# labgem/pangenomeNEM

Hardware: AMD Instinct MI355X
Metric: em_family_x_organism_cells_per_sec (higher is better)
Workload: dtype f32 chains with f64 intermediates (reference arithmetic); int32 popcounts in the M-step; 1 GPU; BASELINE configs[1]: 20000 families x 500 organisms, K=3, beta=0.5, contiguity graph (path + 5% chords, weights 1..8), ncem/sk_/pk; U-shaped family-frequency spectrum (Beta(0.3, 0.3) per family), default .m init; families_total=20000, families_per_gpu=20000, organisms=500, K=3, parallelism=1 GPU

## Files before the change

pangenomenem_amd/csrc/nem_engine.hip:

```cpp
#include <hip/hip_runtime.h>
#include <dlfcn.h>
#include <pthread.h>
#include <unistd.h>

#include <algorithm>
#include <climits>
#include <atomic>
#include <cfloat>
#include <chrono>
#include <cmath>
#include <cstdio>
#include <cstdlib>
#include <cstring>
#include <condition_variable>
#include <deque>
#include <functional>
#include <map>
#include <string>
#include <mutex>
#include <thread>
#include <vector>

#include "nem_internal.hpp"
#include "nem_ff.hpp"
// ... 142 lines not shown
    int* stats_last = nullptr;
    float* par_copy[3] = {}; double* pkfki_copy[3] = {}; float* logpkfki_copy[3] = {};
    int round_batch = 3;
    int rounds_iter = 2;
    int deep_iters = 2;
    uint8_t fz_need[kFzPositions] = {}; uint8_t fz_init_need = 0;
    int run_deep_used = 0; bool run_tracked = false;
    bool capture_first = false;
    int n_plain = 0, n_captured = 0, n_replayed = 0, n_host_rounds = 0;
    int ff_mode = -1;
    bool fused_update() const
    {
        return d <= kFusedMaxD && (cfg.disper == NEMGPU_DISP_KD || cfg.disper == NEMGPU_DISP_K_);
    }
    bool use_ff() const { return ff_mode < 0 ? d >= 256 : ff_mode != 0; }
    bool fault_seen = false; int fault_inject = 0;

    hipEvent_t ev0 = nullptr, ev1 = nullptr;
    hipEvent_t ev_flags = nullptr;
    bool defer_layout = false, layout_pending = false;
    hipEvent_t ready_ev = nullptr;
    bool ready_pending = false;

    struct Chunk { char* base; size_t size, used; bool owned = true; };
    std::vector<Chunk> chunks;
    int shared_chunk = -1;
    uint8_t* best_lab = nullptr; float* best_c = nullptr;
    uint32_t* xf_stage = nullptr;
    bool ctrl_pending = false; CtrlArgs ctrl_deferred{};
    nemgpu_engine* parent = nullptr;
// ... 386 lines not shown
FinishArgs finish_args(nemgpu_engine* e, int mode, const int* stats)
{
    FinishArgs t;
    t.mode = mode;
    t.K = e->k; t.D = e->d; t.dpad = e->dpad; t.n_total = e->n_true; t.disper = e->cfg.disper; t.propor = e->cfg.propor;
    t.stats = stats; t.stats_ranks = 1; t.stats_rank_stride = 0;
    t.prop = e->prop; t.center = e->center; t.disp = e->disp; t.nbobs_k = e->nbobs_k; t.iner = e->iner;
    t.tabT = e->tabT; t.tabL0 = e->tabL0; t.nz0 = e->nz0; t.nz1 = e->nz1;
    t.am0 = e->am0; t.am1 = e->am1; t.uni = e->uni; t.nonuni = e->nonuni;
    t.pk = e->pk; t.logpk = e->logpk; t.flags = e->iter_flags();
    t.stop = e->stop_ptr;
    t.reset_prop = nullptr; t.reset_center = nullptr; t.reset_disp = nullptr;
    t.reset_ctrl = nullptr; t.reset_ctrl_words = 0; t.reset_sweep_next = nullptr;
    t.prev_center = nullptr; t.prev_disp = nullptr;
    t.zero_stats = nullptr; t.n_zero_stats = 0;
    t.use_ff = e->use_ff() ? 1 : 0;
    t.perm = e->perm;
    t.ffq = e->ffq;
    return t;
}

int do_tables(nemgpu_engine* e)
{
    if (e->tables_fresh) return NEMGPU_OK;
    launch_finish(finish_args(e, 0, nullptr), e->stream);
    HIPCHK(hipGetLastError());
    e->tables_fresh = true;
    e->density_fresh = false;
    return NEMGPU_OK;
}

// ... 1626 lines not shown
    e->wf = (d + 31) / 32;
    e->nw64 = (e->n + 63) / 64;
    e->cfg.algo = NEMGPU_ALGO_NCEM; e->cfg.beta = 0.5f; e->cfg.disper = NEMGPU_DISP_K_; e->cfg.propor = NEMGPU_PROP_K;
    e->cfg.cvtest = NEMGPU_CV_CLAS; e->cfg.cvthres = 1e-8f; e->cfg.it_max = 100; e->cfg.param_fix = 0;
    e->cfg.tie_rule = NEMGPU_TIE_HASH; e->cfg.tie_seed = 0;
    if (const char* g = getenv("NEM_MI355X_GRAPHS")) e->use_graphs = (g[0] != '0');
    if (const char* g = getenv("NEM_MI355X_SHADOW_VERIFY")) e->shadow_verify = (g[0] != '0');
    e->flag_sets = e->shadow_verify ? 3 : 1;
    if (const char* g = getenv("NEM_MI355X_ROUND_COUNTS")) e->round_counts = (g[0] != '0');
    if (const char* g = getenv("NEM_MI355X_START_FUSED")) e->start_fused = (g[0] != '0');
    if (const char* g = getenv("NEM_MI355X_ROUNDS")) e->round_batch = std::max(2, std::min(kRoundBatchMax, atoi(g)));
    if (const char* g = getenv("NEM_MI355X_ROUNDS_ITER")) e->rounds_iter = std::max(2, std::min(e->round_batch, atoi(g)));
    e->rounds_iter = std::min(e->rounds_iter, e->round_batch);
    if (const char* g = getenv("NEM_MI355X_FAULT_INJECT")) e->fault_inject = !strcmp(g, "fuzzy_pc") ? 1 : 0;
    if (const char* g = getenv("NEM_MI355X_FF")) e->ff_mode = (g[0] == '0') ? 0 : (g[0] == '1') ? 1 : -1;
    if (const char* g = getenv("NEM_MI355X_SORT")) e->use_sort = (g[0] != '0');
    if (hip_stream) { e->stream = (hipStream_t)hip_stream; e->own_stream = false; }
    else {
        if (pool_stream_get(device, &e->stream) != hipSuccess) { delete e; set_error("hipStreamCreate failed"); return NEMGPU_E_DEVICE; }
        e->own_stream = true;
    }
    int r = NEMGPU_OK;
    alloc_for(e);
    auto A = [&](int rr) { if (r == NEMGPU_OK) r = rr; };
    A(dev_alloc(&e->xw, (size_t)e->W * e->npad));
    A(dev_alloc(&e->xws, (size_t)((e->W + 3) / 4) * 4 * e->npad));
    A(dev_alloc(&e->perm, (size_t)e->npad));
    A(dev_alloc(&e->xt, (size_t)d * e->nw64));
    A(alloc_model_buffers(e));
    if (r == NEMGPU_OK && !e->flags_host &&
// ... 1612 lines not shown
    }
    if (best_start) *best_start = best;
    cleanup();
    return NEMGPU_OK;
}

static int make_clone(nemgpu_engine* p, nemgpu_engine** out, char* slab, size_t slab_bytes, int* flags_host, float* par0)
{
    nemgpu_engine* c = new nemgpu_engine();
    c->n_total = p->n_total; c->n_true = p->n_true; c->d = p->d; c->k = p->k; c->lo = p->lo; c->hi = p->hi; c->n = p->n;
    c->npad = p->npad; c->dpad = p->dpad; c->W = p->W; c->wf = p->wf; c->nw64 = p->nw64; c->device = p->device;
    c->stream = p->stream; c->own_stream = false;
    c->cfg = p->cfg; c->have_matrix = true; c->have_params = true; c->has_graph = p->has_graph;
    c->xw = p->xw; c->xws = p->xws; c->perm = p->perm; c->xt = p->xt; c->use_sort = p->use_sort;
    c->nei_ptr = p->nei_ptr; c->nei_idx = p->nei_idx; c->nei_w = p->nei_w; c->nnz = p->nnz;
    c->use_graphs = p->use_graphs; c->ff_mode = p->ff_mode; c->round_batch = p->round_batch; c->rounds_iter = p->rounds_iter;
    c->parent = p; c->carve_all = true;
    c->chunks.push_back({slab, slab_bytes, 0, false});
    c->shared_chunk = 0;
    c->flags_host = flags_host; c->flags_host_borrowed = true;
    const size_t kd = (size_t)p->k * p->d;
    c->prop0 = par0; c->center0 = par0 + p->k; c->disp0 = par0 + p->k + kd;
    alloc_for(c);
    int r = alloc_model_buffers(c);
    if (r == NEMGPU_OK) r = ensure_state_buffers(c);
    if (r == NEMGPU_OK) r = ensure_crit_buffers(c);
    alloc_for(p);
    if (r != NEMGPU_OK) { nemgpu_destroy(c); return r; }
    c->draw_ctl = c->sweep_next + 8;
    *out = c;
    return NEMGPU_OK;
// ... 63 lines not shown
        if (!e->libc()) { *out = rng.integer(mini, maxi); return NEMGPU_OK; }
        uint32_t v = 0;
        int rr = host_draw(e, &v);
        *out = (int)(v % (uint32_t)(maxi - mini + 1)) + mini;
        return rr;
    };
    auto bit = [&](int i, int j) { return (float)((e->host_bits[(size_t)i * wf + (j >> 5)] >> (j & 31)) & 1u); };
    alloc_for(e);
    if (e->ncem()) { if (!e->best_lab && (r = dev_alloc(&e->best_lab, (size_t)e->n_total))) return r; }
    else { if (!e->best_c && (r = dev_alloc(&e->best_c, (size_t)e->n_total * k))) return r; }
    const int group = std::min(n_starts, 64);
    const char* fa = getenv("NEM_MI355X_STARTS_FIRST_ALONE");
    int width = (e->libc() && !(fa && fa[0] == '0') && fn == nullptr) ? 1 : group;
    int voided_in_a_row = 0, clean_run = 0; bool alone_for_good = false;
    if ((r = ensure_clones(e, group))) return r;
    for (nemgpu_engine* c : e->clones) { c->cfg = e->cfg; c->stream = e->stream; c->round_batch = e->round_batch; c->ff_mode = e->ff_mode; }

    e->rs_rounds = e->rs_lockstep = e->rs_alone = e->rs_redone = e->rs_two_waits = 0;
    if (e->libc()) e->tie_heavy = true;
    int nbsucc = 0, best = -1, last_status = NEMGPU_OK;
    float best_crit[6] = {0, 0, 0, 0, 0, 0};
    nemgpu_result best_res{};
    std::vector<float> host_par;
    std::vector<int> start_pos;
    std::vector<GlibcRandom> rng_after;
    int next = 0;
    static const bool prof = getenv("NEM_MI355X_BATCH_PROF") != nullptr;
    while (next < n_starts) {
        const int M = std::min(width, n_starts - next);
        std::vector<nemgpu_engine*> E(e->clones.begin(), e->clones.begin() + M);
        host_par.assign((size_t)M * par, 0.0f);
// ... 1284 lines not shown
```

pangenomenem_amd/csrc/nem_kernels.hip:

```cpp
#include <hip/hip_runtime.h>
#include <cstdlib>
#include <algorithm>
#include <cfloat>
#include <cstdint>
#include <cstring>
#include <type_traits>

#include "nem_ff.hpp"
#include "nem_chain.hpp"
#include "nem_halfsum.hpp"
#include "nem_kernels.hpp"
#include "nem_sweep_dev.hpp"

namespace nemk {

#ifdef NEM_PHASE_PROF
__device__ unsigned long long g_phase[32];
#define NEM_PHASE(i) do { if (blockIdx.x == 0 && threadIdx.x == 0) g_phase[i] = wall_clock64(); } while (0)
#define NEM_PHASE_TAKE(t) const unsigned long long t = wall_clock64()
#define NEM_PHASE_PUT(i, t) do { if (blockIdx.x == 0 && threadIdx.x == 0) g_phase[i] = t; } while (0)
#else
#define NEM_PHASE(i) do { } while (0)
#define NEM_PHASE_TAKE(t) do { } while (0)
#define NEM_PHASE_PUT(i, t) do { } while (0)
#endif


__device__ __forceinline__ int stat_sum(const int* __restrict__ stats, int idx, int ranks, int stride)
{
    int s = stats[idx];
    for (int r = 1; r < ranks; r++) s += stats[idx + r * stride];
    return s;
}

__device__ inline int wave_reduce_add(int v)
{
// ... 234 lines not shown
    const uint32_t hi = ((mm >> j) & 1u) << 30;
    const double f = __hiloint2double((int)hi, 0);
    return __float_as_uint((float)(fma(f, l1h, (double)__uint_as_float(bits)) - l0));
}

__device__ __forceinline__ void ff_word(uint32_t& bits, uint32_t& q0, uint32_t& dq, uint32_t& end, uint32_t m, int nb,
                                        const uint32_t* sQ0, const uint32_t* sDQ, double l1h, double l0)
{
    const uint32_t cand = ff_cand(m, dq, (nb == 32) ? bits + (q0 << 5) : mad24((uint32_t)nb, q0, bits));
    const bool cross = cand >= end;
    bits = cross ? bits : cand;
    if (cross) {
        uint32_t mm = m;
        int rem = nb;
        for (;;) {
            uint32_t j = 0, at = bits;
#pragma unroll
            for (int sh = 4; sh >= 0; sh--) {
                const uint32_t t = j + (1u << sh);
                const uint32_t at_t = at + (q0 << sh);
                const bool fits = ff_probe(mm, t, dq, at_t) < end;
                j = fits ? t : j;
                at = fits ? at_t : at;
            }
            bits = ff_probe(mm, j, dq, at);
            bits = ff_exact_step(bits, mm, j, l1h, l0);
            ff_load(sQ0, sDQ, bits, q0, dq, end);
            rem -= (int)j + 1;
            if (rem <= 0) break;
            mm = mm >> (j + 1u);
// ... 52 lines not shown
    if (g < gfull) { ff_group(x0, g, am, bits, q0, q1, end, sQ0, sQ1, l1h, l0); xt = x1; g++; }
    if (g < gfull) { ff_group(x1, g, am, bits, q0, q1, end, sQ0, sQ1, l1h, l0); xt = x2; g++; }
    if (g < gfull) { ff_group(x2, g, am, bits, q0, q1, end, sQ0, sQ1, l1h, l0); xt = x3; g++; }
#pragma unroll
    for (int c = 0; c < 4; c++) {
        const int w = 4 * gfull + c;
        if (w > wlast) break;
        uint32_t m = mismatch_word(word_of(xt, c), am[w]);
        const int nb = (w < wlast) ? 32 : (D - (wlast << 5));
        if (nb < 32) m &= (1u << nb) - 1u;
        ff_word(bits, q0, q1, end, m, nb, sQ0, sQ1, l1h, l0);
    }
    return __uint_as_float(bits);
}

__device__ __forceinline__ void ff_build(uint32_t* sQ0, uint32_t* sDQ, double l1, double l0, int tid)
{
    uint32_t q0, q1;
    ff_entry(l1, -l0, tid, q0, q1);
    if (q0 == kFFInvalid) q1 = kFFInvalid;
    sQ0[tid] = q0; sDQ[tid] = q1 - q0;
}

__device__ __forceinline__ void density_store(const int* __restrict__ perm, int slot, int tile, int tid, int n, int npad, int k,
                                              float dk, uint32_t nul, double pk, float logpk,
                                              double* __restrict__ pkfki, float* __restrict__ logpkfki)
{
    __shared__ double sPk[256];
    __shared__ float sLp[256];
    float logfk; double fk;
// ... 99 lines not shown
    const float* center_in; const float* disp_in;
    int* iter_flags;
    double* pkfki; float* logpkfki;
    int* zero_flags; int n_zero_flags;
    int* zero_stats; int n_zero_stats;
    const int* stop;
    int use_ff;
    const int* perm;
};

struct StartArgs {
    const float* prop0; const float* center0; const float* disp0;
    int* ctrl; int ctrl_words; int* sweep_next;
};

template <bool START = false>
__device__ __forceinline__ int density_fused_body(const FusedDensityArgs& a, const StartArgs* st = nullptr)
{
    __shared__ __align__(16) float sVal[FD_MAXD];
    __shared__ double2 sT[FD_CH];
    __shared__ double sL[FD_CH];
    __shared__ uint2 sAm[FD_MAXD / 32];
    __shared__ uint32_t sNz0[FD_CH / 32], sNz1[FD_CH / 32];
    __shared__ uint32_t sQ0[256], sQ1[256];
    __shared__ unsigned long long sTot2w[4];
    __shared__ float sChain[2];
    __shared__ int sGenW[4];
    int k, tile;
    if (!density_tile(a.K, a.npad >> 8, tile, k)) return -1;
    const int tid = threadIdx.x, lane = tid & 63;
    const int i = tile * 256 + tid;
// ... 149 lines not shown
    uint32_t nul = 0;
    bool uniform = !eps_per_d && !any_general && ((double)eps_u > kEpsilonD);
    double l1 = 0.0, l0 = 0.0;
    if (uniform) {
        l1 = log((double)((1.0f - eps_u) / eps_u));
        l0 = log((double)(1.0f - eps_u));
        if (!isfinite(l1) || !isfinite(l0)) uniform = false;
    }
    if (uniform) {
        const double l1h = 0.5 * l1;
        if (a.use_ff && l1 >= 0.0 && l0 <= 0.0) {
            ff_build(sQ0, sQ1, l1, l0, tid);
            __syncthreads();
            NEM_PHASE(21);
            if constexpr (START) xh = xw_head(a.xw, npad, i, D);
            dk = chain_ff(xh, npad, D, sAm, sQ0, sQ1, l1h, l0);
        } else {
            if constexpr (START) xh = xw_head(a.xw, npad, i, D);
            dk = chain_plain(a.xw, xh, npad, i, D, sAm, l1h, l0);
        }
        NEM_PHASE(22);
    } else {
        const bool by_mask = nonempty && !any_general;
        const float* mu_in = START ? st->center0 : a.center_in;
        for (int d0 = 0; d0 < dpad; d0 += FD_CH) {
            const int dn = min(FD_CH, dpad - d0);
            __syncthreads();
            for (int t = tid; t < dn; t += 256) {
                const int d = d0 + t;
                double t0 = 0.0, t1 = 0.0, ll0 = 0.0;
                int n0 = 0, n1 = 0;
// ... 1168 lines not shown
bool launch_halfsum_debug(const float* x, int n, int waves, float* out, hipStream_t s, long long* stamps)
{
    if (n < 0 || n > kHalfsumDebugCap) return false;
    if (waves == 16) hipLaunchKernelGGL(k_halfsum_debug<16>, dim3(1), dim3(1024), 0, s, x, n, out, stamps);
    else if (waves == 1) hipLaunchKernelGGL(k_halfsum_debug<1>, dim3(1), dim3(64), 0, s, x, n, out, stamps);
    else return false;
    return true;
}


__global__ __launch_bounds__(1024) void k_finish(FinishArgs a) { finish_body(a, gridDim.x); }
__global__ __launch_bounds__(1024) void k_finish_b(const void* arr, int stride, const int* gx) { NEM_B_HEAD(FinishArgs) finish_body(a, nblk); }
__global__ __launch_bounds__(256) void k_density(DensityArgs a) { density_body(a); }
__global__ __launch_bounds__(256) void k_density_b(const void* arr, int stride, const int* gx) { NEM_B_HEAD(DensityArgs) density_body(a); }
__global__ __launch_bounds__(256) void k_density_fused(FusedDensityArgs a) { (void)density_fused_body(a); }
__global__ __launch_bounds__(256) void k_density_fused_b(const void* arr, int stride, const int* gx) { NEM_B_HEAD(FusedDensityArgs) (void)density_fused_body(a); }
__global__ __launch_bounds__(256) void k_density_start(FusedDensityArgs a, StartArgs st) { (void)density_fused_body<true>(a, &st); }
template <int KT, int R>
__global__ __launch_bounds__(256) void k_sweep_counts(SweepArgs s, CountsArgs c, int nsweep)
{
    if ((int)blockIdx.x < nsweep) { sweep_body<KT, true, 256, false>(s, blockIdx.x, nsweep); return; }
    mstep_counts_body<R>(c.K, c.D, c.nw64, c.xt, c.mask, c.stats, c.stop, CtrlArgs{}, (int)blockIdx.x - nsweep, (int)gridDim.x - nsweep);
}

template <int KT>
__global__ __launch_bounds__(256) void k_density_verify(FusedDensityArgs d, SweepArgs s, int nd)
{
    if ((int)blockIdx.x < nd) { (void)density_fused_body(d); return; }
    sweep_body<KT, true, 256, false>(s, (int)blockIdx.x - nd, (int)gridDim.x - nd);
}

__global__ void k_ctrl(CtrlArgs a) { ctrl_logic(a); }
// ... 133 lines not shown
    hipLaunchKernelGGL(k_finish, grid, dim3(1024), 0, s, a);
}

void launch_density(const FinishArgs& t, const uint32_t* xw, int n, int npad, double* pkfki, float* logpkfki,
                    int* zero_flags, int n_zero_flags, hipStream_t s)
{
    DensityArgs a;
    a.xw = (const uint4*)xw; a.n = n; a.npad = npad; a.dpad = t.dpad; a.D = t.D; a.K = t.K;
    a.tabT = t.tabT; a.tabL0 = t.tabL0; a.nz0 = t.nz0; a.nz1 = t.nz1; a.am0 = t.am0; a.am1 = t.am1;
    a.uni = t.uni; a.nonuni = t.nonuni; a.pk = t.pk; a.logpk = t.logpk;
    a.pkfki = pkfki; a.logpkfki = logpkfki; a.zero_flags = zero_flags; a.n_zero_flags = n_zero_flags;
    a.stop = t.stop; a.use_ff = t.use_ff; a.perm = t.perm; a.ffq = t.ffq;
    const dim3 grid(((npad / 256 + 7) / 8) * 8 * t.K);
    if (record_op(OP_DENSITY, 0, grid, 256, a)) return;
    hipLaunchKernelGGL(k_density, grid, dim3(256), 0, s, a);
}

static FusedDensityArgs fused_density_args(const FinishArgs& t, const uint32_t* xw, int n, int npad, double* pkfki,
                                           float* logpkfki, int* zero_flags, int n_zero_flags)
{
    FusedDensityArgs a;
    a.xw = (const uint4*)xw; a.n = n; a.npad = npad; a.dpad = t.dpad; a.D = t.D; a.K = t.K; a.n_total = t.n_total;
    a.disper = t.disper; a.propor = t.propor; a.stats = t.stats;
    a.stats_ranks = t.stats_ranks; a.stats_rank_stride = t.stats_rank_stride;
    a.center = t.center; a.disp = t.disp; a.prop = t.prop; a.nbobs_k = t.nbobs_k; a.iter_flags = t.flags;
    a.center_in = t.prev_center != nullptr ? t.prev_center : t.center;
    a.disp_in = t.prev_disp != nullptr ? t.prev_disp : t.disp;
    a.pkfki = pkfki; a.logpkfki = logpkfki; a.zero_flags = zero_flags; a.n_zero_flags = n_zero_flags; a.stop = t.stop;
    a.zero_stats = t.zero_stats; a.n_zero_stats = t.zero_stats != nullptr ? t.n_zero_stats : 0;
    a.use_ff = t.use_ff; a.perm = t.perm;
    return a;
}

void launch_density_fused(const FinishArgs& t, const uint32_t* xw, int n, int npad, double* pkfki, float* logpkfki,
                          int* zero_flags, int n_zero_flags, hipStream_t s)
{
    const FusedDensityArgs a = fused_density_args(t, xw, n, npad, pkfki, logpkfki, zero_flags, n_zero_flags);
    const dim3 grid(((npad / 256 + 7) / 8) * 8 * t.K);
    if (record_op(OP_DENSITY_FUSED, 0, grid, 256, a)) return;
    hipLaunchKernelGGL(k_density_fused, grid, dim3(256), 0, s, a);
}

void launch_density_start(const FinishArgs& t, const uint32_t* xw, int n, int npad, double* pkfki, float* logpkfki,
                          int* zero_flags, int n_zero_flags, hipStream_t s)
{
    const FusedDensityArgs a = fused_density_args(t, xw, n, npad, pkfki, logpkfki, zero_flags, n_zero_flags);
    StartArgs st;
    st.prop0 = t.reset_prop; st.center0 = t.reset_center; st.disp0 = t.reset_disp;
    st.ctrl = t.reset_ctrl; st.ctrl_words = t.reset_ctrl_words; st.sweep_next = t.reset_sweep_next;
    const dim3 grid(((npad / 256 + 7) / 8) * 8 * t.K);
    hipLaunchKernelGGL(k_density_start, grid, dim3(256), 0, s, a, st);
}

bool density_verify_supported(int n_local, int K, int tie_rule)
{
    return n_local < 65536 && K >= 1 && K <= 10 && tie_rule != NEMGPU_TIE_LIBC;
}

void launch_density_verify(const FinishArgs& t, const uint32_t* xw, int n, int npad, double* pkfki, float* logpkfki,
                           int* zero_flags, int n_zero_flags, const SweepArgs& sw, hipStream_t s)
{
    const FusedDensityArgs a = fused_density_args(t, xw, n, npad, pkfki, logpkfki, zero_flags, n_zero_flags);
    const int nd = ((npad / 256 + 7) / 8) * 8 * t.K;
    const int ns = (sw.n_local + 255) / 256;
    const dim3 grid(nd + ns);
#define NEM_DV(KT_) case KT_: hipLaunchKernelGGL((k_density_verify<KT_>), grid, dim3(256), 0, s, a, sw, nd); break;
    switch (sw.K) { NEM_DV(1) NEM_DV(2) NEM_DV(3) NEM_DV(4) NEM_DV(5) NEM_DV(6) NEM_DV(7) NEM_DV(8) NEM_DV(9) NEM_DV(10) default: break; }
#undef NEM_DV
}

bool launch_sweep_counts(const SweepArgs& sw, int K, int D, int nw64, const uint64_t* xt, const uint64_t* mask, int* stats,
                         const int* stop, hipStream_t s)
{
    if (current_recorder() != nullptr || sw.n_local >= 65536 || K < 2 || K > 5 || sw.tie_rule == NEMGPU_TIE_LIBC) return false;
    CountsArgs c{K, D, nw64, xt, mask, stats, stop, CtrlArgs{}};
    const int nsweep = (sw.n_local + 255) / 256;
    const bool wide = D + 1 >= 1024;
    const dim3 grid(nsweep + (wide ? (D + 1 + 3) / 4 : D + 1));
#define NEM_SC(KT_) case KT_:                                                                                        \
        if (wide) hipLaunchKernelGGL((k_sweep_counts<KT_, 4>), grid, dim3(256), 0, s, sw, c, nsweep);                \
        else hipLaunchKernelGGL((k_sweep_counts<KT_, 1>), grid, dim3(256), 0, s, sw, c, nsweep);                     \
// ... 113 lines not shown
        acc ^= v.x ^ v.y ^ v.z ^ v.w;
    }
    if (acc == 0x9E3779B9u) sink[0] = acc;
}

void launch_calib_read(const uint32_t* buf, size_t words, uint32_t* sink, hipStream_t s)
{
    hipLaunchKernelGGL(k_calib_read16, dim3(256 * 16), dim3(256), 0, s, (const uint4*)buf, words / 4, sink);
}

#ifdef NEM_PHASE_PROF
extern "C" int nemgpu_debug_phases(unsigned long long* out32)
{
    return (int)hipMemcpyFromSymbol(out32, HIP_SYMBOL(g_phase), sizeof(unsigned long long) * 32);
}
#endif

}
```

pangenomenem_amd/csrc/nem_kernels.hpp:

```cpp
#pragma once
#include <hip/hip_runtime.h>
#include <cstdint>
#include <cstring>
#include <type_traits>
#include <vector>

#include "../../include/nem_mi355x.h"

namespace nemk {

constexpr int kMaxKernelK = 32;
constexpr int kTicketWords = 32 * 33;
constexpr double kEpsilonD = 1e-20;

enum { FLAG_CHANGED = 0, FLAG_NZERO = 1, FLAG_FIRSTZERO = 2, FLAG_NTIES = 3, FLAG_ROUND_STRIDE = 4 };
enum { FLAG_EMPTYK = 0, FLAG_EMPTY_PROP = 1, FLAG_FAULT = 2, FLAG_MOVED = 3, FLAG_ITER_STRIDE = 4 };

enum { C_STOP = 0, C_FOLD = 1, C_ITERS = 10, C_COMMITS = 2, C_STATUS = 3, C_EMPTYK = 4, C_CONVERGED = 5, C_NEED_ROUNDS = 6,
       C_SWEEP_ROUNDS = 7, C_NZERO = 8, C_FIRSTZERO = 9, C_DRAWS = 11, C_DEEP = 12, C_DRAWS_INIT = 13, C_INIT_ROUNDS = 14, C_WORDS = 16 };

struct CtrlArgs {
    int* ctrl; const int* iter_flags; const int* round0;
    int n_rounds;
    int param_fix, use_nei, cvtest, ncem; float cvthres;
// ... 86 lines not shown
    uint32_t* am0; uint32_t* am1; double2* uni; int* nonuni;
    double* pk; float* logpk; int* flags;
    const int* stop;
    const float* reset_prop; const float* reset_center; const float* reset_disp;
    int* reset_ctrl; int reset_ctrl_words; int* reset_sweep_next;
    const int* perm;
    int use_ff;
    uint2* ffq;
    const float* prev_center; const float* prev_disp;
    int* zero_stats; int n_zero_stats;
};
void launch_finish(const FinishArgs& a, hipStream_t s);
void launch_density(const FinishArgs& t, const uint32_t* xw, int n, int npad, double* pkfki, float* logpkfki,
                    int* zero_flags, int n_zero_flags, hipStream_t s);
constexpr int kFusedMaxD = 1024;
void launch_density_fused(const FinishArgs& t, const uint32_t* xw, int n, int npad, double* pkfki, float* logpkfki,
                          int* zero_flags, int n_zero_flags, hipStream_t s);
void launch_density_start(const FinishArgs& t, const uint32_t* xw, int n, int npad, double* pkfki, float* logpkfki,
                          int* zero_flags, int n_zero_flags, hipStream_t s);
bool density_verify_supported(int n_local, int K, int tie_rule);
void launch_density_verify(const FinishArgs& t, const uint32_t* xw, int n, int npad, double* pkfki, float* logpkfki,
                           int* zero_flags, int n_zero_flags, const SweepArgs& sw, hipStream_t s);
void launch_sweep(const SweepArgs& a, bool ncem, hipStream_t s);
bool launch_sweep_counts(const SweepArgs& sw, int K, int D, int nw64, const uint64_t* xt, const uint64_t* mask, int* stats,
                         const int* stop, hipStream_t s);
void launch_labels_post(int n_local, int lo, int K, int nw64, const uint8_t* lab_new, const uint8_t* lab_old,
                        uint64_t* mask, int* flags, const int* stop, const CtrlArgs* ctrl, hipStream_t s);
void launch_mstep_counts(int K, int D, int nw64, const uint64_t* xt, const uint64_t* mask, int* stats,
                         const int* stop, const CtrlArgs* prev_ctrl, hipStream_t s);
void launch_mstep_fuzzy(int n, int npad, int K, int D, const uint32_t* xw, const uint64_t* xt, int nw64, const float* c,
// ... 36 lines not shown
```

Baseline: 353.3 billion cells/s.

## Add wave-batched fast-forward chain walker with shared-memory mismatch rows

Adds a batched variant of the fast-forward Bernoulli chain in the fused density kernel. Each lane's mismatch words are staged in dynamic shared memory. Lanes advance word by word several steps per decision, and the costly exact crossing search runs only once enough lanes in a wave are waiting or none can advance. It is on by default when D>32 and the grid is small relative to the CU count, and it keeps the old word-synchronous kernel as a fallback. The aim is to cut wave divergence from per-word crossing loops; the cost is about 35 KB of dynamic shared memory per block plus extra ballots and branches.

New measurement: 376.4 billion cells/s (median of 6 runs). 6.5% higher.

```diff
diff --git a/pangenomenem_amd/csrc/nem_engine.hip b/pangenomenem_amd/csrc/nem_engine.hip
--- a/pangenomenem_amd/csrc/nem_engine.hip
+++ b/pangenomenem_amd/csrc/nem_engine.hip
@@ -180,6 +180,7 @@
         return d <= kFusedMaxD && (cfg.disper == NEMGPU_DISP_KD || cfg.disper == NEMGPU_DISP_K_);
     }
     bool use_ff() const { return ff_mode < 0 ? d >= 256 : ff_mode != 0; }
+    bool ff_batch = true;
     bool fault_seen = false; int fault_inject = 0;
 
     hipEvent_t ev0 = nullptr, ev1 = nullptr;
@@ -596,7 +597,7 @@
     t.reset_ctrl = nullptr; t.reset_ctrl_words = 0; t.reset_sweep_next = nullptr;
     t.prev_center = nullptr; t.prev_disp = nullptr;
     t.zero_stats = nullptr; t.n_zero_stats = 0;
-    t.use_ff = e->use_ff() ? 1 : 0;
+    t.use_ff = !e->use_ff() ? FF_OFF : e->ff_batch ? FF_BATCHED : FF_WORD;
     t.perm = e->perm;
     t.ffq = e->ffq;
     return t;
@@ -2253,6 +2254,7 @@
     e->rounds_iter = std::min(e->rounds_iter, e->round_batch);
     if (const char* g = getenv("NEM_MI355X_FAULT_INJECT")) e->fault_inject = !strcmp(g, "fuzzy_pc") ? 1 : 0;
     if (const char* g = getenv("NEM_MI355X_FF")) e->ff_mode = (g[0] == '0') ? 0 : (g[0] == '1') ? 1 : -1;
+    if (const char* g = getenv("NEM_MI355X_FF_BATCH")) e->ff_batch = (g[0] != '0');
     if (const char* g = getenv("NEM_MI355X_SORT")) e->use_sort = (g[0] != '0');
     if (hip_stream) { e->stream = (hipStream_t)hip_stream; e->own_stream = false; }
     else {
@@ -3895,7 +3897,7 @@
     c->cfg = p->cfg; c->have_matrix = true; c->have_params = true; c->has_graph = p->has_graph;
     c->xw = p->xw; c->xws = p->xws; c->perm = p->perm; c->xt = p->xt; c->use_sort = p->use_sort;
     c->nei_ptr = p->nei_ptr; c->nei_idx = p->nei_idx; c->nei_w = p->nei_w; c->nnz = p->nnz;
-    c->use_graphs = p->use_graphs; c->ff_mode = p->ff_mode; c->round_batch = p->round_batch; c->rounds_iter = p->rounds_iter;
+    c->use_graphs = p->use_graphs; c->ff_mode = p->ff_mode; c->ff_batch = p->ff_batch; c->round_batch = p->round_batch; c->rounds_iter = p->rounds_iter;
     c->parent = p; c->carve_all = true;
     c->chunks.push_back({slab, slab_bytes, 0, false});
     c->shared_chunk = 0;
@@ -3989,7 +3991,7 @@
     int width = (e->libc() && !(fa && fa[0] == '0') && fn == nullptr) ? 1 : group;
     int voided_in_a_row = 0, clean_run = 0; bool alone_for_good = false;
     if ((r = ensure_clones(e, group))) return r;
-    for (nemgpu_engine* c : e->clones) { c->cfg = e->cfg; c->stream = e->stream; c->round_batch = e->round_batch; c->ff_mode = e->ff_mode; }
+    for (nemgpu_engine* c : e->clones) { c->cfg = e->cfg; c->stream = e->stream; c->round_batch = e->round_batch; c->ff_mode = e->ff_mode; c->ff_batch = e->ff_batch; }
 
     e->rs_rounds = e->rs_lockstep = e->rs_alone = e->rs_redone = e->rs_two_waits = 0;
     if (e->libc()) e->tie_heavy = true;
diff --git a/pangenomenem_amd/csrc/nem_kernels.hip b/pangenomenem_amd/csrc/nem_kernels.hip
--- a/pangenomenem_amd/csrc/nem_kernels.hip
+++ b/pangenomenem_amd/csrc/nem_kernels.hip
@@ -19,7 +19,13 @@
 #define NEM_PHASE(i) do { if (blockIdx.x == 0 && threadIdx.x == 0) g_phase[i] = wall_clock64(); } while (0)
 #define NEM_PHASE_TAKE(t) const unsigned long long t = wall_clock64()
 #define NEM_PHASE_PUT(i, t) do { if (blockIdx.x == 0 && threadIdx.x == 0) g_phase[i] = t; } while (0)
+__device__ unsigned long long g_ff_wave[12];
+#define NEM_FF_WAVE_ADD(slot, v) do { if (blockIdx.x == 0 && (int)__lane_id() == __ffsll((unsigned long long)__ballot(1)) - 1) \
+        atomicAdd(&g_ff_wave[4 * (slot) + (threadIdx.x >> 6)], (unsigned long long)(v)); } while (0)
+#define NEM_FF_WAVE_END() do { if (blockIdx.x == 0 && (threadIdx.x & 63) == 0) g_ff_wave[threadIdx.x >> 6] = wall_clock64(); } while (0)
 #else
+#define NEM_FF_WAVE_ADD(slot, v) do { } while (0)
+#define NEM_FF_WAVE_END() do { } while (0)
 #define NEM_PHASE(i) do { } while (0)
 #define NEM_PHASE_TAKE(t) do { } while (0)
 #define NEM_PHASE_PUT(i, t) do { } while (0)
@@ -284,6 +290,7 @@
         uint32_t mm = m;
         int rem = nb;
         for (;;) {
+            NEM_FF_WAVE_ADD(2, 1);
             uint32_t j = 0, at = bits;
 #pragma unroll
             for (int sh = 4; sh >= 0; sh--) {
@@ -366,6 +373,108 @@
     return __uint_as_float(bits);
 }
 
+#ifndef NEM_FF_BATCH_T
+#define NEM_FF_BATCH_T 16
+#endif
+#ifndef NEM_FF_BATCH_STEPS
+#define NEM_FF_BATCH_STEPS 3
+#endif
+constexpr int kFFBatchT = NEM_FF_BATCH_T;
+constexpr int kFFBatchSteps = NEM_FF_BATCH_STEPS;
+constexpr int kFFRowWords = kFusedMaxD / 32 + 3;
+static_assert(kFFPlainSteps == 32, "chain_ff_batched steps the whole first word");
+
+__device__ __forceinline__ float chain_ff_batched(const XwHead& h, int npad, int D, uint32_t* sRow, const uint2* am,
+                                                  const uint32_t* sQ0, const uint32_t* sDQ, double l1h, double l0)
+{
+    const int tid = threadIdx.x;
+    const int wlast = (D - 1) >> 5;
+    const int glast = wlast >> 2;
+    uint32_t* row = sRow + tid;
+    auto put = [&](const int g, const uint4& v) {
+        row[(4 * g + 0) * 256] = mismatch_word(v.x, am[4 * g + 0]); row[(4 * g + 1) * 256] = mismatch_word(v.y, am[4 * g + 1]);
+        row[(4 * g + 2) * 256] = mismatch_word(v.z, am[4 * g + 2]); row[(4 * g + 3) * 256] = mismatch_word(v.w, am[4 * g + 3]);
+    };
+    uint4 y0 = h.x0, y1 = h.x0, y2 = h.x0, y3 = h.x0;
+    {
+        const uint4* p = h.pn;
+        if (glast >= 4) y0 = *p;
+        if (glast >= 5) y1 = p[npad];
+        if (glast >= 6) y2 = p[2 * (size_t)npad];
+        if (glast >= 7) y3 = p[3 * (size_t)npad];
+    }
+    uint32_t bits, q0, dq, end;
+    {
+        const uint32_t m = mismatch_word(h.x0.x, am[0]);
+        float dk0 = 0.0f;
+#pragma unroll
+        for (int b = 0; b < 32; b++) dk0 = bern_step(dk0, m, b, l1h, l0);
+        bits = __float_as_uint(dk0);
+        ff_load(sQ0, sDQ, bits, q0, dq, end);
+    }
+    put(0, h.x0);
+    if (glast >= 1) put(1, h.x1);
+    if (glast >= 2) put(2, h.x2);
+    if (glast >= 3) put(3, h.x3);
+    if (glast >= 4) put(4, y0);
+    if (glast >= 5) put(5, y1);
+    if (glast >= 6) put(6, y2);
+    if (glast >= 7) put(7, y3);
+    const uint32_t nlast = (uint32_t)(D - (wlast << 5));
+    int w = 1;
+    uint32_t mm = row[256];
+    uint32_t rem = (wlast == 1) ? nlast : 32u;
+    uint32_t mn = row[2 * 256], mn2 = row[3 * 256];
+    auto advance = [&](const bool take) {
+        w += take ? 1 : 0;
+        mm = take ? mn : mm;
+        mn = take ? mn2 : mn;
+        rem = take ? ((w == wlast) ? nlast : 32u) : rem;
+        mn2 = row[(w + 2) * 256];
+    };
+    for (;;) {
+        const bool active = w <= wlast;
+        const uint32_t cand = ff_cand(mm, dq, mad24(rem, q0, bits));
+        const bool fits = active && cand < end;
+        const uint64_t bact = __builtin_amdgcn_ballot_w64(active);
+        if (bact == 0) break;
+        const uint64_t ba = __builtin_amdgcn_ballot_w64(fits);
+        NEM_FF_WAVE_ADD(1, 1);
+        bits = fits ? cand : bits;
+        bool take = fits;
+        if (__popcll(bact & ~ba) >= kFFBatchT || ba == 0) {
+            NEM_FF_WAVE_ADD(2, 1);
+            if (active && !fits) {
+                uint32_t j = 0, at = bits;
+#pragma unroll
+                for (int sh = 4; sh >= 0; sh--) {
+                    const uint32_t t = j + (1u << sh);
+                    const uint32_t at_t = at + (q0 << sh);
+                    const bool ok = ff_probe(mm, t, dq, at_t) < end;
+                    j = ok ? t : j;
+                    at = ok ? at_t : at;
+                }
+                bits = ff_probe(mm, j, dq, at);
+                bits = ff_exact_step(bits, mm, j, l1h, l0);
+                ff_load(sQ0, sDQ, bits, q0, dq, end);
+                rem -= j + 1u;
+                mm = (mm >> j) >> 1;
+                take = (rem == 0u);
+            }
+        }
+        advance(take);
+#pragma unroll
+        for (int s = 1; s < kFFBatchSteps; s++) {
+            const uint32_t c2 = ff_cand(mm, dq, mad24(rem, q0, bits));
+            const bool f2 = (w <= wlast) && c2 < end;
+            NEM_FF_WAVE_ADD(1, 1);
+            bits = f2 ? c2 : bits;
+            advance(f2);
+        }
+    }
+    return __uint_as_float(bits);
+}
+
 __device__ __forceinline__ void ff_build(uint32_t* sQ0, uint32_t* sDQ, double l1, double l0, int tid)
 {
     uint32_t q0, q1;
@@ -495,7 +604,7 @@
     int* ctrl; int ctrl_words; int* sweep_next;
 };
 
-template <bool START = false>
+template <bool START = false, bool ROW = true>
 __device__ __forceinline__ int density_fused_body(const FusedDensityArgs& a, const StartArgs* st = nullptr)
 {
     __shared__ __align__(16) float sVal[FD_MAXD];
@@ -675,7 +784,16 @@
             __syncthreads();
             NEM_PHASE(21);
             if constexpr (START) xh = xw_head(a.xw, npad, i, D);
-            dk = chain_ff(xh, npad, D, sAm, sQ0, sQ1, l1h, l0);
+            bool walked = false;
+            if constexpr (ROW) {
+                extern __shared__ uint32_t sRow[];
+                if (a.use_ff == FF_BATCHED) {
+                    dk = chain_ff_batched(xh, npad, D, sRow, sAm, sQ0, sQ1, l1h, l0);
+                    walked = true;
+                }
+            }
+            if (!walked) dk = chain_ff(xh, npad, D, sAm, sQ0, sQ1, l1h, l0);
+            NEM_FF_WAVE_END();
         } else {
             if constexpr (START) xh = xw_head(a.xw, npad, i, D);
             dk = chain_plain(a.xw, xh, npad, i, D, sAm, l1h, l0);
@@ -1874,8 +1992,10 @@
 __global__ __launch_bounds__(256) void k_density(DensityArgs a) { density_body(a); }
 __global__ __launch_bounds__(256) void k_density_b(const void* arr, int stride, const int* gx) { NEM_B_HEAD(DensityArgs) density_body(a); }
 __global__ __launch_bounds__(256) void k_density_fused(FusedDensityArgs a) { (void)density_fused_body(a); }
-__global__ __launch_bounds__(256) void k_density_fused_b(const void* arr, int stride, const int* gx) { NEM_B_HEAD(FusedDensityArgs) (void)density_fused_body(a); }
+__global__ __launch_bounds__(256) void k_density_fused_b(const void* arr, int stride, const int* gx) { NEM_B_HEAD(FusedDensityArgs) (void)density_fused_body<false, false>(a); }
 __global__ __launch_bounds__(256) void k_density_start(FusedDensityArgs a, StartArgs st) { (void)density_fused_body<true>(a, &st); }
+__global__ __launch_bounds__(256) void k_density_fused_word(FusedDensityArgs a) { (void)density_fused_body<false, false>(a); }
+__global__ __launch_bounds__(256) void k_density_start_word(FusedDensityArgs a, StartArgs st) { (void)density_fused_body<true, false>(a, &st); }
 template <int KT, int R>
 __global__ __launch_bounds__(256) void k_sweep_counts(SweepArgs s, CountsArgs c, int nsweep)
 {
@@ -2039,6 +2159,21 @@
     const dim3 grid(((npad / 256 + 7) / 8) * 8 * t.K);
     if (record_op(OP_DENSITY, 0, grid, 256, a)) return;
     hipLaunchKernelGGL(k_density, grid, dim3(256), 0, s, a);
+}
+
+static int density_blocks(int npad, int K) { return ((npad / 256 + 7) / 8) * 8 * K; }
+
+static int compute_units()
+{
+    static int cus[64] = {};
+    int dev = 0;
+    if (hipGetDevice(&dev) != hipSuccess || dev < 0 || dev >= 64) return 0;
+    if (cus[dev] == 0) {
+        int v = 0;
+        if (hipDeviceGetAttribute(&v, hipDeviceAttributeMultiprocessorCount, dev) != hipSuccess || v <= 0) return 0;
+        cus[dev] = v;
+    }
+    return cus[dev];
 }
 
 static FusedDensityArgs fused_density_args(const FinishArgs& t, const uint32_t* xw, int n, int npad, double* pkfki,
@@ -2054,7 +2189,13 @@
     a.pkfki = pkfki; a.logpkfki = logpkfki; a.zero_flags = zero_flags; a.n_zero_flags = n_zero_flags; a.stop = t.stop;
     a.zero_stats = t.zero_stats; a.n_zero_stats = t.zero_stats != nullptr ? t.n_zero_stats : 0;
     a.use_ff = t.use_ff; a.perm = t.perm;
+    if (a.use_ff == FF_BATCHED && !(t.D > 32 && density_blocks(npad, t.K) <= 3 * compute_units())) a.use_ff = FF_WORD;
     return a;
+}
+
+static size_t ff_row_bytes(const FusedDensityArgs& a)
+{
+    return a.use_ff == FF_BATCHED ? sizeof(uint32_t) * kFFRowWords * 256 : 0;
 }
 
 void launch_density_fused(const FinishArgs& t, const uint32_t* xw, int n, int npad, double* pkfki, float* logpkfki,
@@ -2063,7 +2204,8 @@
     const FusedDensityArgs a = fused_density_args(t, xw, n, npad, pkfki, logpkfki, zero_flags, n_zero_flags);
     const dim3 grid(((npad / 256 + 7) / 8) * 8 * t.K);
     if (record_op(OP_DENSITY_FUSED, 0, grid, 256, a)) return;
-    hipLaunchKernelGGL(k_density_fused, grid, dim3(256), 0, s, a);
+    if (a.use_ff == FF_BATCHED) hipLaunchKernelGGL(k_density_fused, grid, dim3(256), ff_row_bytes(a), s, a);
+    else hipLaunchKernelGGL(k_density_fused_word, grid, dim3(256), 0, s, a);
 }
 
 void launch_density_start(const FinishArgs& t, const uint32_t* xw, int n, int npad, double* pkfki, float* logpkfki,
@@ -2074,7 +2216,8 @@
     st.prop0 = t.reset_prop; st.center0 = t.reset_center; st.disp0 = t.reset_disp;
     st.ctrl = t.reset_ctrl; st.ctrl_words = t.reset_ctrl_words; st.sweep_next = t.reset_sweep_next;
     const dim3 grid(((npad / 256 + 7) / 8) * 8 * t.K);
-    hipLaunchKernelGGL(k_density_start, grid, dim3(256), 0, s, a, st);
+    if (a.use_ff == FF_BATCHED) hipLaunchKernelGGL(k_density_start, grid, dim3(256), ff_row_bytes(a), s, a, st);
+    else hipLaunchKernelGGL(k_density_start_word, grid, dim3(256), 0, s, a, st);
 }
 
 bool density_verify_supported(int n_local, int K, int tie_rule)
@@ -2089,7 +2232,7 @@
     const int nd = ((npad / 256 + 7) / 8) * 8 * t.K;
     const int ns = (sw.n_local + 255) / 256;
     const dim3 grid(nd + ns);
-#define NEM_DV(KT_) case KT_: hipLaunchKernelGGL((k_density_verify<KT_>), grid, dim3(256), 0, s, a, sw, nd); break;
+#define NEM_DV(KT_) case KT_: hipLaunchKernelGGL((k_density_verify<KT_>), grid, dim3(256), ff_row_bytes(a), s, a, sw, nd); break;
     switch (sw.K) { NEM_DV(1) NEM_DV(2) NEM_DV(3) NEM_DV(4) NEM_DV(5) NEM_DV(6) NEM_DV(7) NEM_DV(8) NEM_DV(9) NEM_DV(10) default: break; }
 #undef NEM_DV
 }
@@ -2233,6 +2376,10 @@
 {
     return (int)hipMemcpyFromSymbol(out32, HIP_SYMBOL(g_phase), sizeof(unsigned long long) * 32);
 }
+extern "C" int nemgpu_debug_ff_waves(unsigned long long* out12)
+{
+    return (int)hipMemcpyFromSymbol(out12, HIP_SYMBOL(g_ff_wave), sizeof(unsigned long long) * 12);
+}
 #endif
 
 }
diff --git a/pangenomenem_amd/csrc/nem_kernels.hpp b/pangenomenem_amd/csrc/nem_kernels.hpp
--- a/pangenomenem_amd/csrc/nem_kernels.hpp
+++ b/pangenomenem_amd/csrc/nem_kernels.hpp
@@ -124,6 +124,7 @@
 void launch_density(const FinishArgs& t, const uint32_t* xw, int n, int npad, double* pkfki, float* logpkfki,
                     int* zero_flags, int n_zero_flags, hipStream_t s);
 constexpr int kFusedMaxD = 1024;
+enum FFMode { FF_OFF = 0, FF_WORD = 1, FF_BATCHED = 2 };
 void launch_density_fused(const FinishArgs& t, const uint32_t* xw, int n, int npad, double* pkfki, float* logpkfki,
                           int* zero_flags, int n_zero_flags, hipStream_t s);
 void launch_density_start(const FinishArgs& t, const uint32_t* xw, int n, int npad, double* pkfki, float* logpkfki,
diff --git a/profiles/ff_batch_phases.py b/profiles/ff_batch_phases.py
--- /dev/null
+++ b/profiles/ff_batch_phases.py
@@ -0,0 +1,82 @@
+#!/usr/bin/env python3
+import argparse
+import ctypes as C
+import json
+import os
+import statistics
+import sys
+import tempfile
+
+ROOT = os.path.dirname(os.path.dirname(os.path.abspath(__file__)))
+sys.path.insert(0, ROOT)
+sys.path.insert(0, os.path.dirname(os.path.abspath(__file__)))
+
+LAUNCHES = 8
+
+
+def main():
+    from entry_loads_phases import DENSITY, build_instrumented
+    ap = argparse.ArgumentParser()
+    ap.add_argument("--dir", default=None)
+    ap.add_argument("--build-only", action="store_true")
+    ap.add_argument("--cycles", type=int, default=20)
+    ap.add_argument("--out", default=None)
+    args = ap.parse_args()
+    where = args.dir or tempfile.mkdtemp(prefix="nem_phase_prof_")
+    os.makedirs(where, exist_ok=True)
+    lib_path = build_instrumented(where)
+    print("instrumented library:", lib_path, file=sys.stderr)
+    if args.build_only:
+        return 0
+    os.environ["NEM_MI355X_LIB"] = lib_path
+    os.environ["NEM_MI355X_GRAPHS"] = "0"
+    import bench
+    from pangenomenem_amd.engine import load_library
+    lib = load_library()
+    lib.nemgpu_debug_phases.argtypes = [C.POINTER(C.c_ulonglong)]
+    lib.nemgpu_debug_ff_waves.argtypes = [C.POINTER(C.c_ulonglong)]
+    x, nei, prop, center, disp, disper, _ = bench.make_workload(20000, 500, 3, "ushape", 2)
+    run = bench.EngineRun(x, nei, 3, prop, center, disp, "ncem", 0.5, "sk_", tie="hash")
+    run.prime(run.cycle * 4, run.cycle)
+
+    def waves():
+        v = (C.c_ulonglong * 12)()
+        if lib.nemgpu_debug_ff_waves(v) != 0:
+            raise RuntimeError("nemgpu_debug_ff_waves")
+        return [int(t) for t in v]
+    dens, ends, steps, passes = [], [], [], []
+    before = waves()
+    for _ in range(args.cycles):
+        run.run_steps(run.cycle)
+        d = (C.c_ulonglong * 32)()
+        if lib.nemgpu_debug_phases(d) != 0:
+            return 1
+        now = waves()
+        dens.append([(int(d[i]) - int(d[16])) / 100.0 for i, _ in DENSITY])
+        ends.append([(now[j] - int(d[16])) / 100.0 for j in range(4)])
+        steps.append([(now[4 + j] - before[4 + j]) / LAUNCHES for j in range(4)])
+        passes.append([(now[8 + j] - before[8 + j]) / LAUNCHES for j in range(4)])
+        before = now
+    run.eng.close()
+
+    def med(rows):
+        return [statistics.median(r[j] for r in rows) for j in range(len(rows[0]))]
+    phase = dict(zip((name for _, name in DENSITY), med(dens)))
+    end = med(ends)
+    out = {"unit": "us since block 0's entry, median over %d restart cycles (100 MHz clock: 0.01 us steps)" % args.cycles,
+           "chain": "word-synchronous" if os.environ.get("NEM_MI355X_FF_BATCH", "1")[0] == "0" else "batched",
+           "density_fused_body": phase,
+           "chain_end_per_wave": end,
+           "slowest_wave_chain_us": round(max(end) - phase["ff tables (behind their barrier)"], 2),
+           "store_behind_slowest_wave_us": round(phase["stored"] - max(end), 2),
+           "lane_steps_per_wave_and_launch": med(steps), "passes_per_wave_and_launch": med(passes)}
+    text = json.dumps(out, indent=1)
+    print(text)
+    if args.out:
+        with open(args.out, "w") as f:
+            f.write(text + "\n")
+    return 0
+
+
+if __name__ == "__main__":
+    sys.exit(main())
diff --git a/profiles/ff_schedule_model.py b/profiles/ff_schedule_model.py
--- /dev/null
+++ b/profiles/ff_schedule_model.py
@@ -0,0 +1,214 @@
+#!/usr/bin/env python3
+import argparse
+import ctypes as C
+import json
+import os
+import sys
+
+import numpy as np
+
+ROOT = os.path.dirname(os.path.dirname(os.path.abspath(__file__)))
+sys.path.insert(0, ROOT)
+
+SLOTS_STEPPED, SLOTS_WORD, SLOTS_TRIP, SLOTS_PASS = 192, 10, 14, 80
+INVALID = 1 << 23
+
+
+def popc(v):
+    v = v.astype(np.uint64)
+    v = v - ((v >> 1) & 0x55555555)
+    v = (v & 0x33333333) + ((v >> 2) & 0x33333333)
+    v = (v + (v >> 4)) & 0x0F0F0F0F
+    return ((v * 0x01010101) & 0xFFFFFFFF) >> 24
+
+
+class Chain:
+
+    def __init__(self, lib, eps):
+        e = np.float32(eps)
+        self.l1 = float(np.log(np.float64((np.float32(1.0) - e) / e)))
+        self.l0 = float(np.log(np.float64(np.float32(1.0) - e)))
+        q0 = (C.c_uint32 * 256)(); q1 = (C.c_uint32 * 256)()
+        assert lib.nemgpu_ff_table(C.c_double(self.l1), C.c_double(self.l0), q0, q1) == 0
+        q0 = np.array(list(q0), np.uint64); q1 = np.array(list(q1), np.uint64)
+        q1[q0 == INVALID] = INVALID
+        self.Q0, self.DQ = q0, q1 - q0
+        self.usable = self.l1 >= 0.0 and self.l0 <= 0.0
+
+    def load(self, bits):
+        E = (bits >> np.uint64(23)) & np.uint64(255)
+        return self.Q0[E], self.DQ[E], (E + np.uint64(1)) << np.uint64(23)
+
+    def exact(self, bits, bit):
+        dk = bits.astype(np.uint32).view(np.float32).astype(np.float64)
+        r = ((dk + np.where(bit != 0, self.l1, 0.0)) - self.l0).astype(np.float32)
+        return r.view(np.uint32).astype(np.uint64)
+
+    def stepped_word(self, m):
+        bits = np.zeros(len(m), np.uint64)
+        for b in range(32):
+            bits = self.exact(bits, (m >> np.uint64(b)) & np.uint64(1))
+        return bits
+
+    def cross(self, bits, q0, dq, end, mm, rem):
+        j = np.zeros(len(bits), np.uint64); at = bits.copy()
+        for sh in (4, 3, 2, 1, 0):
+            t = j + np.uint64(1 << sh)
+            at_t = at + (q0 << np.uint64(sh))
+            low = mm & ((np.uint64(1) << t) - np.uint64(1))
+            ok = at_t + popc(low) * dq < end
+            j = np.where(ok, t, j); at = np.where(ok, at_t, at)
+        assert np.all(j < rem)
+        low = mm & ((np.uint64(1) << j) - np.uint64(1))
+        bits = self.exact(at + popc(low) * dq, (mm >> j) & np.uint64(1))
+        q0, dq, end = self.load(bits)
+        return bits, q0, dq, end, mm >> (j + np.uint64(1)), rem - (j + np.uint64(1))
+
+
+def word_synchronous(ch, M, nbs, wave):
+    nw = int(wave.max()) + 1
+    passes = np.zeros(nw, np.int64)
+    bits = ch.stepped_word(M[:, 0])
+    q0, dq, end = ch.load(bits)
+    for w in range(1, M.shape[1]):
+        m = M[:, w].copy(); nb = np.uint64(nbs[w])
+        cand = bits + nb * q0 + popc(m) * dq
+        crossing = cand >= end
+        bits = np.where(crossing, bits, cand)
+        idx = np.flatnonzero(crossing)
+        mm = m[idx]; rem = np.full(len(idx), nb, np.uint64)
+        while len(idx):
+            passes[np.unique(wave[idx])] += 1
+            b, a, d, e, mm, rem = ch.cross(bits[idx], q0[idx], dq[idx], end[idx], mm, rem)
+            c2 = b + rem * a + popc(mm) * d
+            done = (rem == 0) | (c2 < e)
+            b = np.where((rem > 0) & (c2 < e), c2, b)
+            bits[idx], q0[idx], dq[idx], end[idx] = b, a, d, e
+            idx, mm, rem = idx[~done], mm[~done], rem[~done]
+    return bits, np.full(nw, M.shape[1] - 1, np.int64), passes
+
+
+def batched(ch, M, nbs, wave, T, S=1):
+    n, W = M.shape
+    nw = int(wave.max()) + 1
+    trips = np.zeros(nw, np.int64); passes = np.zeros(nw, np.int64)
+    bits = ch.stepped_word(M[:, 0])
+    q0, dq, end = ch.load(bits)
+    w = np.ones(n, np.int64)
+    mm = M[:, 1].copy(); rem = np.full(n, nbs[1], np.uint64)
+    nbs = np.asarray(list(nbs) + [0], np.uint64)
+    Mx = np.concatenate([M, np.zeros((n, 1), np.uint64)], axis=1)
+    rows = np.arange(n)
+    step = 0
+    while True:
+        active = w < W
+        decide = step % S == 0
+        if decide and not active.any():
+            break
+        step += 1
+        cand = bits + rem * q0 + popc(mm) * dq
+        fits = active & (cand < end)
+        waits = active & ~fits
+        nwait = np.bincount(wave[waits], minlength=nw); nadv = np.bincount(wave[fits], minlength=nw)
+        bits = np.where(fits, cand, bits)
+        if decide:
+            trips += S * ((nwait + nadv) > 0)
+            run = (nwait >= T) | ((nadv == 0) & (nwait > 0))
+        else:
+            run = np.zeros(nw, bool)
+        passes += run
+        idx = np.flatnonzero(waits & run[wave])
+        take = fits.copy()
+        if len(idx):
+            b, a, d, e, m2, r2 = ch.cross(bits[idx], q0[idx], dq[idx], end[idx], mm[idx], rem[idx])
+            bits[idx], q0[idx], dq[idx], end[idx], mm[idx], rem[idx] = b, a, d, e, m2, r2
+            take[idx] = r2 == 0
+        w = w + take
+        wc = np.minimum(w, W)
+        mm = np.where(take, Mx[rows, wc], mm); rem = np.where(take, nbs[wc], rem)
+    return bits, trips, passes
+
+
+def summary(units, passes, slots_unit):
+    slots = SLOTS_STEPPED + slots_unit * units + SLOTS_PASS * passes
+    nb = len(slots) // 4
+    blk = slots[:nb * 4].reshape(nb, 4).max(axis=1)
+    return {"units_per_wave_mean_max": [round(float(units.mean()), 2), int(units.max())],
+            "passes_per_wave_mean_max": [round(float(passes.mean()), 2), int(passes.max())],
+            "slots_mean_wave": round(float(slots.mean())), "slots_slowest_wave_per_block_median": round(float(np.median(blk))),
+            "slots_worst_wave": int(slots.max())}
+
+
+def main():
+    ap = argparse.ArgumentParser()
+    ap.add_argument("--out", default=None)
+    ap.add_argument("--iterations", default="0,1,2,4,7")
+    ap.add_argument("--thresholds", default="16,32,48,64")
+    ap.add_argument("--steps", default="1,3", help="lane steps per wave decision")
+    ap.add_argument("--families", type=int, default=20000)
+    ap.add_argument("--organisms", type=int, default=500)
+    args = ap.parse_args()
+    from oracle.pyoracle import Oracle
+    from pangenomenem_amd import build, synth
+    from pangenomenem_amd.engine import load_library
+    build.build()
+    lib = load_library()
+    lib.nemgpu_ff_table.argtypes = [C.c_double, C.c_double, C.POINTER(C.c_uint32), C.POINTER(C.c_uint32)]
+    n, d, k = args.families, args.organisms, 3
+    x, _ = synth.ushaped_pa_matrix(n, d, 2)
+    nei = synth.contiguity_graph(n, 2, d=d)
+    start = synth.default_init(d)
+    orc = Oracle()
+    W = (d + 31) // 32
+    nbs = [32] * (W - 1) + [d - 32 * (W - 1)]
+    xp = np.zeros((n, W * 32), np.uint8); xp[:, :d] = x
+    xw = (xp.reshape(n, W, 32).astype(np.uint64) << np.arange(32, dtype=np.uint64)).sum(axis=2)
+    pc = x.sum(axis=1)
+    perm = np.concatenate([t0 + np.argsort(pc[t0:t0 + 256], kind="stable") for t0 in range(0, n, 256)])
+    wave = np.arange(n) // 64
+    out = {"shape": [n, d, k], "slots": {"stepped_word": SLOTS_STEPPED, "word": SLOTS_WORD, "trip": SLOTS_TRIP, "pass": SLOTS_PASS},
+           "units": "word-synchronous: words; batched: lane steps (S per wave decision, each priced as a trip)", "iterations": {}}
+    for it in [int(v) for v in args.iterations.split(",")]:
+        if it == 0:
+            prop, center, disp = start
+        else:
+            r = orc.run(x, nei, k, *start, algo="ncem", beta=0.5, disper="sk_", cvtest="none", it_max=it, tie="hash")
+            prop, center, disp = r["prop"], r["center"], r["disp"]
+        _, lp, _ = orc.density(x, prop, center, disp)
+        res = {}
+        for c in range(k):
+            eps = float(disp[c, 0])
+            assert np.all(disp[c] == disp[c, 0]) and set(np.unique(center[c])) <= {0.0, 0.5, 1.0}
+            ch = Chain(lib, eps)
+            a0 = np.abs((0.0 - center[c]).astype(np.int32)) != 0; a1 = np.abs((1.0 - center[c]).astype(np.int32)) != 0
+            mis = np.where(xp[:, :d] != 0, a1[None, :], a0[None, :]).astype(np.uint8)
+            mp = np.zeros((n, W * 32), np.uint8); mp[:, :d] = mis
+            M = (mp.reshape(n, W, 32).astype(np.uint64) << np.arange(32, dtype=np.uint64)).sum(axis=2)[perm]
+            logpk = np.float32(np.log(np.float64(prop[c])))
+            want = lp[perm, c]
+
+            def held(bits):
+                got = logpk + (-bits.astype(np.uint32).view(np.float32))
+                return bool(np.array_equal(got.view(np.uint32), want.view(np.uint32)))
+            rc = {"epsilon": eps}
+            bits, units, passes = word_synchronous(ch, M, nbs, wave)
+            rc["word_synchronous"] = dict(summary(units, passes, SLOTS_WORD), oracle_bits=held(bits))
+            for S in [int(v) for v in args.steps.split(",")]:
+                for T in [int(v) for v in args.thresholds.split(",")]:
+                    bits, units, passes = batched(ch, M, nbs, wave, T, S)
+                    rc["batched_T%d_S%d" % (T, S)] = dict(summary(units, passes, SLOTS_TRIP), oracle_bits=held(bits))
+            res["class_%d" % c] = rc
+            print("iteration", it, "class", c, json.dumps(rc), file=sys.stderr, flush=True)
+        out["iterations"][str(it)] = res
+    text = json.dumps(out, indent=1)
+    if args.out:
+        with open(args.out, "w") as f:
+            f.write(text + "\n")
+    else:
+        print(text)
+    return 0 if all(v["oracle_bits"] for r in out["iterations"].values() for c in r.values()
+                    for v in c.values() if isinstance(v, dict)) else 1
+
+
+if __name__ == "__main__":
+    sys.exit(main())
```
